# Vincentqyw/image-matching-webui

Measured on AMD Instinct MI355X. Metric: image-pairs/sec @640x480 SuperPoint+LightGlue, higher is better.
Workload: dtype f32 via 3xf16 split MFMA, f32 accumulate; P.V of LightGlue's cross blocks in two products (audited per block: layer error <= 7.1e-6, score error <= 4.7e-5, profiles/r05_lab_attention_mix.txt)

## Files before the change

image-matching-webui_amd/csrc/api.hip:

```cpp
#include <stdarg.h>
#include <stdio.h>
#include <stdlib.h>
#include <string.h>

#include "attention.h"
#include "conv.h"
#include "ffn.h"
#include "gemm.h"
#include "imcui_hip.h"

int imcui_set_err(imcui_hip_s* h, int code, const char* fmt, ...) {
    if (h) {
        va_list ap;
        va_start(ap, fmt);
        vsnprintf(h->err, sizeof h->err, fmt, ap);
        va_end(ap);
    }
    return code;
}

extern "C" int imcui_hip_version(void) { return 400; }

static const char* const OPT_NAMES[OPT_NCNT] = {"gemm_wreg", "wreg_pipe", "attn_variant", "attn_variant_self", "attn_variant_cross", "attn_mix_layers", "conv_tall", "conv_narrow", "simred", "ffn_tile", "wreg_tile", "attn_split", "loftr_fine_sparse"};
static int opt_index(const char* name) {
    if (!name) return -1;
    for (int i = 0; i < OPT_NCNT; ++i)
        if (strcmp(name, OPT_NAMES[i]) == 0) return i;
    return -1;
}
extern "C" int imcui_hip_set_option(imcui_hip_t* h, const char* name, int value) {
    const int i = opt_index(name);
    if (!h || i < 0) return imcui_set_err(h, IMCUI_ERR_ARG, "set_option: unknown option '%s'", name ? name : "(null)");
    h->opt[i] = value;
    return IMCUI_OK;
}
extern "C" int imcui_hip_get_option(imcui_hip_t* h, const char* name, int* value) {
    const int i = opt_index(name);
    if (!h || !value || i < 0) return imcui_set_err(h, IMCUI_ERR_ARG, "get_option: unknown option '%s'", name ? name : "(null)");
    *value = h->opt[i];
    return IMCUI_OK;
}

extern "C" int imcui_hip_create(int device, imcui_hip_t** out) {
    if (!out) return IMCUI_ERR_ARG;
    *out = nullptr;
    int n = 0;
    if (hipGetDeviceCount(&n) != hipSuccess || device < 0 || device >= n) return IMCUI_ERR_HIP;
    hipDeviceProp_t prop;
    if (hipGetDeviceProperties(&prop, device) != hipSuccess) return IMCUI_ERR_HIP;
    imcui_hip_s* h = (imcui_hip_s*)calloc(1, sizeof(imcui_hip_s));
    if (!h) return IMCUI_ERR_ARG;
    h->device = device;
    h->num_cu = prop.multiProcessorCount;
    h->err[0] = 0;
    h->precision = 1;
    {
        const char* e;
        h->opt[OPT_GEMM_WREG] = (e = getenv("IMCUI_GEMM_WREG")) ? atoi(e) : 2;
        h->opt[OPT_WREG_PIPE] = (e = getenv("IMCUI_WREG_PIPE")) ? atoi(e) : 1;
        h->opt[OPT_ATTN_VARIANT] = (e = getenv("IMCUI_ATTN_VARIANT")) ? atoi(e) : 8;
        h->opt[OPT_SIMRED] = (e = getenv("IMCUI_SIMRED")) ? atoi(e) : 1;
        h->opt[OPT_FFN_TILE] = (e = getenv("IMCUI_FFN_TILE")) ? atoi(e) : 0;
        h->opt[OPT_WREG_TILE] = (e = getenv("IMCUI_WREG_TILE")) ? atoi(e) : 0;
        h->opt[OPT_CONV_TALL] = (e = getenv("IMCUI_CONV_TALL")) ? atoi(e) : 1;
        h->opt[OPT_CONV_NARROW] = (e = getenv("IMCUI_CONV_NARROW")) ? atoi(e) : 0;
        h->opt[OPT_ATTN_SELF] = (e = getenv("IMCUI_ATTN_VARIANT_SELF")) ? atoi(e) : -1;
        h->opt[OPT_ATTN_CROSS] = (e = getenv("IMCUI_ATTN_VARIANT_CROSS")) ? atoi(e) : -2;
        h->opt[OPT_ATTN_SPLIT] = (e = getenv("IMCUI_ATTN_SPLIT")) ? atoi(e) : 1;
        h->opt[OPT_LOFTR_FINE_SPARSE] = (e = getenv("IMCUI_LOFTR_FINE_SPARSE")) ? atoi(e) : 1;
        h->opt[OPT_ATTN_MIX_LAYERS] = (e = getenv("IMCUI_ATTN_MIX_LAYERS")) ? (int)strtol(e, nullptr, 0) : 0x1ff;
    }
    *out = h;
    const char* rc = getenv("IMCUI_HIP_CHECK_RANGE");
    if (rc && atoi(rc) != 0) (void)imcui_hip_set_range_check(h, 1);
    return IMCUI_OK;
}

__global__ __launch_bounds__(256) void range_check_kernel(const float* __restrict__ x, long rows, int cols, long ld, const int* __restrict__ cnt,
                                                          int rows_per_seq, int* __restrict__ flag) {
    int bits = 0;
    const long n4 = rows * (long)(cols >> 2);
    for (long t = (long)blockIdx.x * 256 + threadIdx.x; t < n4; t += (long)gridDim.x * 256) {
        const long r = t / (cols >> 2);
        const int c = (int)(t - r * (cols >> 2)) * 4;
        if (cnt != nullptr && rows_per_seq > 0 && (int)(r % rows_per_seq) >= cnt[r / rows_per_seq]) continue;
        const float4 v = *reinterpret_cast<const float4*>(x + r * ld + c);
        const float a[4] = {v.x, v.y, v.z, v.w};
#pragma unroll
        for (int j = 0; j < 4; ++j) {
            if (!(fabsf(a[j]) <= 3.4028234e38f)) bits |= 2;
            else if (fabsf(a[j]) > 65504.0f) bits |= 1;
        }
    }
    if (bits) atomicOr(flag, bits);
}
void imcui_range_check(imcui_hip_s* h, const float* x, long rows, int cols, long ld, const int* cnt, int rows_per_seq, hipStream_t s) {
    if (!h || !h->range_flag || !x || rows <= 0 || cols < 4 || (cols & 3) || (ld & 3)) return;
    const long n4 = rows * (long)(cols >> 2);
// ... 540 lines not shown
```

image-matching-webui_amd/csrc/common.h:

```cpp
#pragma once
#include <hip/hip_runtime.h>
#include <stdint.h>

#include <atomic>

typedef float f32x16 __attribute__((ext_vector_type(16)));
typedef float f32x4 __attribute__((ext_vector_type(4)));

#define IMCUI_WAVE 64

__device__ __forceinline__ f32x16 mfma32(float a, float b, f32x16 c) {
    return __builtin_amdgcn_mfma_f32_32x32x2f32(a, b, c, 0, 0, 0);
}

typedef _Float16 f16x8 __attribute__((ext_vector_type(8)));
typedef _Float16 f16x2 __attribute__((ext_vector_type(2)));
typedef __fp16 fp16x2_t __attribute__((ext_vector_type(2)));

__device__ __forceinline__ f32x16 mfma16(uint4 a, uint4 b, f32x16 c) {
    return __builtin_amdgcn_mfma_f32_32x32x16_f16(__builtin_bit_cast(f16x8, a), __builtin_bit_cast(f16x8, b), c, 0, 0, 0);
}
__device__ __forceinline__ void split2(float x0, float x1, unsigned& hi, unsigned& lo) {
    const fp16x2_t h = __builtin_amdgcn_cvt_pkrtz(x0, x1);
    hi = __builtin_bit_cast(unsigned, h);
// ... 79 lines not shown
    int dev = 0;
    (void)hipGetDevice(&dev);
    const unsigned long long bit = 1ull << (dev & 63);
    if (done.load(std::memory_order_acquire) & bit) return true;
    if (hipFuncSetAttribute(kernel, hipFuncAttributeMaxDynamicSharedMemorySize, bytes) != hipSuccess) return false;
    done.fetch_or(bit, std::memory_order_release);
    return true;
}
static inline int cdiv(int a, int b) { return (a + b - 1) / b; }
static inline size_t align_up(size_t v, size_t a) { return (v + a - 1) / a * a; }
static inline unsigned blocks_256(long n) { return (unsigned)((n + 255) / 256); }
static inline unsigned grid_stride_blocks(long n) { return (n + 255) / 256 < 65536 ? blocks_256(n) : 65536u; }

#define IMCUI_OK 0
#define IMCUI_ERR_ARG -1
#define IMCUI_ERR_WS -2
#define IMCUI_ERR_HIP -3
#define IMCUI_ERR_UNSUPPORTED -4

enum {
    OPT_GEMM_WREG = 0,
    OPT_WREG_PIPE,
    OPT_ATTN_VARIANT,
    OPT_ATTN_SELF,
    OPT_ATTN_CROSS,
    OPT_ATTN_MIX_LAYERS,
    OPT_CONV_TALL,
    OPT_CONV_NARROW,
    OPT_SIMRED,
    OPT_FFN_TILE,
    OPT_WREG_TILE,
    OPT_ATTN_SPLIT,
    OPT_LOFTR_FINE_SPARSE,
    OPT_NCNT
};

#define IMCUI_GEMM_ROUTE_SLOTS 384
#define IMCUI_ATTN_ROUTE_SLOTS 16
#define IMCUI_CONV_ROUTE_SLOTS 16
#define IMCUI_FFN_ROUTE_SLOTS 17

enum { PROF_ATTN = 0, PROF_CONV = 1, PROF_GEMM = 2, PROF_NCLS = 3 };
#define PROF_MAX_EVENTS 4096
struct imcui_hip_s {
    int device;
    int num_cu;
    char err[512];
    int precision;
    int prof_on;
    int prof_used[PROF_NCLS];
    int prof_alloc[PROF_NCLS];
    hipEvent_t* prof_ev[PROF_NCLS];
    float* lg_dump;
    size_t lg_dump_floats;
    long long* ffn_dbg;
    int* range_flag;
    int opt[OPT_NCNT];
    int loftr_fine_mode;
    int loftr_fine_matches;
    int gemm_last_route;
    int gemm_route_count[IMCUI_GEMM_ROUTE_SLOTS];
    int gemm_route_features[IMCUI_GEMM_ROUTE_SLOTS];
    int attn_last_route;
    int attn_route_count[IMCUI_ATTN_ROUTE_SLOTS];
    int conv_last_route;
    int conv_route_count[IMCUI_CONV_ROUTE_SLOTS];
// ... 39 lines not shown
```

image-matching-webui_amd/csrc/conv.hip:

```cpp
#include <stdlib.h>

#include "conv.h"
#include "gemm.h"

#define TH 8
#define TW 16
#define PW (TW + 2)
#define PH (TH + 2)
#define NPIX (PH * PW)
#define PSTR 181
#define WSTR 65

__global__ __launch_bounds__(256) void conv3x3_kernel(const float* __restrict__ in, const float* __restrict__ wp,
                                                      const float* __restrict__ bias, float* __restrict__ out, int H,
                                                      int W, int Cin, int Cout, int tiles_x, int tiles_y, int relu,
                                                      int pool) {
    __shared__ float4 Ps[8 * PSTR];
    __shared__ float4 Ws[2][8 * WSTR];

    const int tid = threadIdx.x, lane = tid & 63, wid = tid >> 6;
    const int lo = lane & 31, hi = lane >> 5;
    const int ncout = Cout >> 6;
    const int t = xcd_remap(blockIdx.x, gridDim.x);
    const int ct = t % ncout;
// ... 81 lines not shown
            }
        }
    }
}

int conv3x3_launch(imcui_hip_s* h, const float* in, const float* wp, const float* bias, float* out, int B, int H, int W,
                   int Cin, int Cout, int relu, int pool, hipStream_t stream) {
    h->conv_last_route = CONV_ROUTE(CR_NONE);
    if (Cin % 32 != 0 || Cout % 64 != 0)
        return imcui_set_err(h, IMCUI_ERR_ARG, "conv3x3: Cin=%d must be a multiple of 32, Cout=%d of 64", Cin, Cout);
    if (pool && ((H | W) & 1)) return imcui_set_err(h, IMCUI_ERR_ARG, "conv3x3: pooled layer needs even H,W (%dx%d)", H, W);
    const int tiles_x = cdiv(W, TW), tiles_y = cdiv(H, TH);
    const long nwg = (long)tiles_x * tiles_y * (Cout / 64) * B;
    if (nwg <= 0) return IMCUI_OK;
    imcui_prof_begin(h, PROF_CONV, stream);
    hipLaunchKernelGGL(conv3x3_kernel, dim3((unsigned)nwg), dim3(256), 0, stream, in, wp, bias, out, H, W, Cin, Cout,
                       tiles_x, tiles_y, relu, pool);
    conv_route_note(h, CR_F32, pool ? CF_POOL : 0);
    imcui_prof_end(h, PROF_CONV, stream);
    IMCUI_CHECK_LAUNCH(h);
    return IMCUI_OK;
}

#define STH 8
#define STW 32
#define SPW (STW + 2)
#define SNPIX ((STH + 2) * SPW)
#define SPSTR 346

#define ITW (STW + 4)
#define ITH (STH + 4)
__device__ __forceinline__ float conv_act(float v, int code) { return code == 2 ? (v > 0.0f ? v : 0.01f * v) : (code == 1 ? fmaxf(v, 0.0f) : v); }

template <bool FUSE1A, int NC, bool SINGLE = false>
__global__ __launch_bounds__(256, NC == 4 ? 2 : 3) void conv3x3_split_kernel(const float* __restrict__ in,
                                                            const unsigned short* __restrict__ wh,
                                                            const unsigned short* __restrict__ wl,
                                                            const float* __restrict__ wscale,
                                                            const float* __restrict__ bias, float* __restrict__ out,
                                                            int H, int W, int Cin, int Cout, int tiles_x, int tiles_y,
                                                            int relu, int pool, const float* __restrict__ w1a,
                                                            const float* __restrict__ b1a, int cin_stride, int cout_live, ConvHead hd) {
    constexpr int WSN = NC * 32 + 1;
    static_assert(NC == 2 || (NC == 4 && !FUSE1A), "the fused first layer has 64 output channels");
    __shared__ uint4 smem[2 * 4 * SPSTR + 2 * 2 * 4 * WSN + (FUSE1A ? (ITH * ITW + 9 * 64 + 64 + 3) / 4 + 1 : 0)];
    uint4* Ph = smem;
    uint4* Pl = smem + 4 * SPSTR;
    uint4* Wb = smem + 2 * 4 * SPSTR;
    float* img = reinterpret_cast<float*>(smem + 2 * 4 * SPSTR + 2 * 2 * 4 * WSN);
    float* w1 = img + ITH * ITW;

    const int tid = threadIdx.x, lane = tid & 63, wid = tid >> 6;
    const int lo = lane & 31, hi = lane >> 5;
    const int ncout = Cout / (32 * NC);
    const int t = xcd_remap(blockIdx.x, gridDim.x);
    const int ct = t % ncout;
    int sp = t / ncout;
    const int tx = sp % tiles_x;
    sp /= tiles_x;
    const int ty = sp % tiles_y;
    const int b = sp / tiles_y;
    const int y0 = ty * STH, x0 = tx * STW, cout0 = ct * 32 * NC;
    const int nlive = min(NC, (cout_live - cout0 + 31) >> 5);
    const bool relu_in = !FUSE1A && (relu & 4) != 0;
    relu &= 3;

    f32x16 acc[2][NC];
#pragma unroll
    for (int m = 0; m < 2; ++m)
#pragma unroll
        for (int n = 0; n < NC; ++n)
#pragma unroll
            for (int r = 0; r < 16; ++r) acc[m][n][r] = 0.0f;

    const int nchunk = Cin >> 5;
    const uint4* wh4 = reinterpret_cast<const uint4*>(wh);
    const uint4* wl4 = reinterpret_cast<const uint4*>(wl);

    if (FUSE1A) {
        for (int i = tid; i < ITH * ITW; i += 256) {
            const int gy = y0 - 2 + i / ITW, gx = x0 - 2 + i % ITW;
            img[i] = (gy >= 0 && gy < H && gx >= 0 && gx < W) ? in[((size_t)b * H + gy) * W + gx] : 0.0f;
        }
        for (int i = tid; i < 9 * 64; i += 256) w1[i] = w1a[i];
        if (tid < 64) w1[9 * 64 + tid] = b1a[tid];
    }

    constexpr int NPG = (SNPIX * 4 + 255) / 256;
    float4 pa[NPG], pc[NPG];
    unsigned pvalid = 0;
    auto patch_fetch = [&](int ch) __attribute__((always_inline)) {
        pvalid = 0;
#pragma unroll
        for (int k = 0; k < NPG; ++k) {
            const int idx = tid + 256 * k;
            const int oc = idx & 3, pp = idx >> 2;
            const int py = pp / SPW, px = pp - py * SPW;
            const int gy = y0 - 1 + py, gx = x0 - 1 + px;
            if (idx < SNPIX * 4 && gy >= 0 && gy < H && gx >= 0 && gx < W) {
                const float* src = in + (((size_t)b * H + gy) * W + gx) * cin_stride + ch * 32 + oc * 8;
                pa[k] = *reinterpret_cast<const float4*>(src);
                pc[k] = *reinterpret_cast<const float4*>(src + 4);
                pvalid |= 1u << k;
            }
        }
    };
    auto patch_store = [&]() __attribute__((always_inline)) {
#pragma unroll
        for (int k = 0; k < NPG; ++k) {
            const int idx = tid + 256 * k;
            if (idx < SNPIX * 4) {
                uint4 hq = make_uint4(0u, 0u, 0u, 0u), lq = hq;
                if ((pvalid >> k) & 1u) {
                    if (relu_in) {
                        pa[k] = make_float4(fmaxf(pa[k].x, 0.f), fmaxf(pa[k].y, 0.f), fmaxf(pa[k].z, 0.f), fmaxf(pa[k].w, 0.f));
                        pc[k] = make_float4(fmaxf(pc[k].x, 0.f), fmaxf(pc[k].y, 0.f), fmaxf(pc[k].z, 0.f), fmaxf(pc[k].w, 0.f));
                    }
                    if constexpr (SINGLE)
                        hq = half8_rtn(pa[k], pc[k]);
                    else
                        split8(pa[k], pc[k], hq, lq);
                }
                Ph[(idx & 3) * SPSTR + (idx >> 2)] = hq;
                if constexpr (!SINGLE) Pl[(idx & 3) * SPSTR + (idx >> 2)] = lq;
            }
        }
    };
    constexpr bool PREFETCH = (NC == 2);
    if (!FUSE1A && PREFETCH) patch_fetch(0);

    for (int ch = 0; ch < nchunk; ++ch) {
        if (!FUSE1A && !PREFETCH) patch_fetch(ch);
        __syncthreads();
        if (!FUSE1A) {
            patch_store();
            if (PREFETCH && ch + 1 < nchunk) patch_fetch(ch + 1);
        }
        float4 kw0[9], kw1[9], kb0, kb1;
        if (FUSE1A) {
            const int c0 = ch * 32 + (tid & 3) * 8;
            kb0 = *reinterpret_cast<const float4*>(w1 + 9 * 64 + c0);
            kb1 = *reinterpret_cast<const float4*>(w1 + 9 * 64 + c0 + 4);
#pragma unroll
            for (int t9 = 0; t9 < 9; ++t9) {
                kw0[t9] = *reinterpret_cast<const float4*>(w1 + t9 * 64 + c0);
                kw1[t9] = *reinterpret_cast<const float4*>(w1 + t9 * 64 + c0 + 4);
            }
        }
        for (int idx = tid; FUSE1A && idx < SNPIX * 4; idx += 256) {
            const int oc = idx & 3, pp = idx >> 2;
            const int py = pp / SPW, px = pp - py * SPW;
            const int gy = y0 - 1 + py, gx = x0 - 1 + px;
            uint4 hq = make_uint4(0u, 0u, 0u, 0u), lq = hq;
            if (gy >= 0 && gy < H && gx >= 0 && gx < W) {
                float4 a, c;
                if (FUSE1A) {
                    a = kb0;
// ... 20 lines not shown
                    c = *reinterpret_cast<const float4*>(src + 4);
                }
                split8(a, c, hq, lq);
            }
            Ph[oc * SPSTR + pp] = hq;
            Pl[oc * SPSTR + pp] = lq;
        }
        uint4 rwh, rwl, rwh1, rwl1;
        auto wload = [&](int tap) __attribute__((always_inline)) {
            const size_t o = ((size_t)(ch * 9 + tap) * 4 + (tid >> 6)) * Cout + cout0 + (tid & 63);
            rwh = wh4[o];
            if constexpr (!SINGLE) rwl = wl4[o];
            if constexpr (NC == 4) {
                rwh1 = wh4[o + 64];
                if constexpr (!SINGLE) rwl1 = wl4[o + 64];
            }
        };
        wload(0);
        for (int tap = 0; tap < 9; ++tap) {
            uint4* wbh = Wb + (tap & 1) * (2 * 4 * WSN);
            uint4* wbl = wbh + 4 * WSN;
            wbh[(tid >> 6) * WSN + (tid & 63)] = rwh;
            if constexpr (!SINGLE) wbl[(tid >> 6) * WSN + (tid & 63)] = rwl;
            if constexpr (NC == 4) {
                wbh[(tid >> 6) * WSN + (tid & 63) + 64] = rwh1;
                if constexpr (!SINGLE) wbl[(tid >> 6) * WSN + (tid & 63) + 64] = rwl1;
            }
            __syncthreads();
            if (tap + 1 < 9) wload(tap + 1);
            const int dy = tap / 3, dx = tap - dy * 3;
#pragma unroll
            for (int st = 0; st < 2; ++st) {
                const int oc = 2 * st + hi;
                uint4 ah[2], al[2], bh[NC], bl[NC];
#pragma unroll
                for (int m = 0; m < 2; ++m) {
                    const int pp = (2 * wid + m + dy) * SPW + lo + dx;
                    ah[m] = Ph[oc * SPSTR + pp];
                    if constexpr (!SINGLE) al[m] = Pl[oc * SPSTR + pp];
                }
#pragma unroll
                for (int n = 0; n < NC; ++n) {
                    bh[n] = wbh[oc * WSN + n * 32 + lo];
                    if constexpr (!SINGLE) bl[n] = wbl[oc * WSN + n * 32 + lo];
                }
#pragma unroll
                for (int n = 0; n < NC; ++n) {
                    if (NC == 4 && n == NC - 1 && nlive < NC) break;
#pragma unroll
                    for (int m = 0; m < 2; ++m) {
                        if constexpr (!SINGLE) {
                            acc[m][n] = mfma16(bh[n], al[m], acc[m][n]);
                            acc[m][n] = mfma16(bl[n], ah[m], acc[m][n]);
                        }
                        acc[m][n] = mfma16(bh[n], ah[m], acc[m][n]);
                    }
                }
            }
        }
    }

    const float wsc = wscale[0];
    const float* resid = FUSE1A ? nullptr : w1a;
    const float* resid2 = FUSE1A ? nullptr : b1a;
    const bool late = resid != nullptr;
    __syncthreads();
    float* st = reinterpret_cast<float*>(smem);
    constexpr int SROW = 68;
#pragma unroll
    for (int half = 0; half < NC / 2; ++half) {
        const int coutH = cout0 + 64 * half;
        if (half > 0) __syncthreads();
        if (pool) {
            const int Ho = H >> 1, Wo = W >> 1;
#pragma unroll
            for (int n = 0; n < 2; ++n)
#pragma unroll
                for (int q = 0; q < 4; ++q) {
                    const int cl = n * 32 + 8 * q + 4 * hi;
                    const float4 b4 = *reinterpret_cast<const float4*>(bias + coutH + cl);
                    float v[4];
#pragma unroll
                    for (int j = 0; j < 4; ++j) {
                        float tv = fmaxf(acc[0][2 * half + n][4 * q + j], acc[1][2 * half + n][4 * q + j]);
                        tv = fmaxf(tv, __shfl_xor(tv, 1, 64));
                        v[j] = tv * wsc;
                    }
                    v[0] += b4.x;
                    v[1] += b4.y;
                    v[2] += b4.z;
                    v[3] += b4.w;
                    if (relu) {
#pragma unroll
                        for (int j = 0; j < 4; ++j) v[j] = conv_act(v[j], relu);
                    }
                    if ((lo & 1) == 0) *reinterpret_cast<float4*>(st + (wid * 16 + (lo >> 1)) * SROW + cl) = make_float4(v[0], v[1], v[2], v[3]);
                }
            __syncthreads();
#pragma unroll
            for (int it = 0; it < 4; ++it) {
                const int px = (tid >> 4) + 16 * it, c4 = tid & 15;
                const int oy = (y0 >> 1) + (px >> 4), pxo = (x0 >> 1) + (px & 15);
                if (oy < Ho && pxo < Wo)
                    *reinterpret_cast<float4*>(out + (((size_t)b * Ho + oy) * Wo + pxo) * Cout + coutH + 4 * c4) =
                        *reinterpret_cast<const float4*>(st + px * SROW + 4 * c4);
            }
        } else {
#pragma unroll
            for (int h2 = 0; h2 < 2; ++h2) {
                if ((wid >> 1) == h2) {
#pragma unroll
                    for (int n = 0; n < 2; ++n)
#pragma unroll
                        for (int q = 0; q < 4; ++q) {
                            const int cl = n * 32 + 8 * q + 4 * hi;
                            const float4 b4 = *reinterpret_cast<const float4*>(bias + coutH + cl);
#pragma unroll
                            for (int m = 0; m < 2; ++m) {
                                float4 v = make_float4(acc[m][2 * half + n][4 * q + 0] * wsc + b4.x, acc[m][2 * half + n][4 * q + 1] * wsc + b4.y,
                                                       acc[m][2 * half + n][4 * q + 2] * wsc + b4.z, acc[m][2 * half + n][4 * q + 3] * wsc + b4.w);
                                if (relu && !late) {
                                    v.x = conv_act(v.x, relu);
                                    v.y = conv_act(v.y, relu);
                                    v.z = conv_act(v.z, relu);
                                    v.w = conv_act(v.w, relu);
                                }
                                *reinterpret_cast<float4*>(st + (((wid & 1) * 2 + m) * 32 + lo) * SROW + cl) = v;
                            }
                        }
                }
                __syncthreads();
                if constexpr (NC == 4 && !FUSE1A) {
                    if (hd.w != nullptr) {
                        const int c4 = tid & 15;
                        float4 hw[4];
#pragma unroll
                        for (int c = 0; c < 4; ++c) hw[c] = *reinterpret_cast<const float4*>(hd.w + c * 128 + 64 * half + 4 * c4);
                        float* psum = st + 128 * SROW;
#pragma unroll
                        for (int it = 0; it < 8; ++it) {
                            const int px = (tid >> 4) + 16 * it;
                            const float4 v = *reinterpret_cast<const float4*>(st + px * SROW + 4 * c4);
                            float d[4];
#pragma unroll
                            for (int c = 0; c < 4; ++c) {
                                d[c] = (v.x * hw[c].x + v.y * hw[c].y) + (v.z * hw[c].z + v.w * hw[c].w);
#pragma unroll
                                for (int o = 8; o > 0; o >>= 1) d[c] += __shfl_xor(d[c], o, 64);
                            }
                            if (c4 == 0) {
                                float4* ps = reinterpret_cast<float4*>(psum + (h2 * 128 + px) * 4);
                                if (half == 0) {
                                    *ps = make_float4(d[0], d[1], d[2], d[3]);
                                } else {
                                    const float4 q = *ps;
                                    const int oy = y0 + 4 * h2 + (px >> 5), ox = x0 + (px & 31);
                                    if (oy < H && ox < W) {
                                        const float x = (q.x + d[0]) + hd.b[0], y = (q.y + d[1]) + hd.b[1], z = (q.z + d[2]) + hd.b[2], cf = (q.w + d[3]) + hd.b[3];
                                        const size_t p = ((size_t)b * H + oy) * W + ox;
                                        if (hd.raw) *reinterpret_cast<float4*>(hd.raw + p * 4) = make_float4(x, y, z, cf);
                                        const float dn = sqrtf(x * x + y * y + z * z);
                                        const float sc = expm1f(dn) / fmaxf(dn, 1e-8f);
                                        hd.pts[p * 3 + 0] = x * sc;
                                        hd.pts[p * 3 + 1] = y * sc;
                                        hd.pts[p * 3 + 2] = z * sc;
                                        hd.conf[p] = 1.0f + expf(cf);
                                    }
                                }
                            }
                        }
                    }
                }
#pragma unroll
                for (int it = 0; it < 8; ++it) {
                    const int px = (tid >> 4) + 16 * it, c4 = tid & 15;
                    const int oy = y0 + 4 * h2 + (px >> 5), ox = x0 + (px & 31);
                    if (oy < H && ox < W && out != nullptr) {
                        float4 v = *reinterpret_cast<const float4*>(st + px * SROW + 4 * c4);
                        const size_t o = (((size_t)b * H + oy) * W + ox) * Cout + coutH + 4 * c4;
                        if (late) {
                            float4 r4 = *reinterpret_cast<const float4*>(resid + o);
                            v = make_float4(v.x + r4.x, v.y + r4.y, v.z + r4.z, v.w + r4.w);
                            if (resid2) {
                                r4 = *reinterpret_cast<const float4*>(resid2 + o);
                                v = make_float4(v.x + r4.x, v.y + r4.y, v.z + r4.z, v.w + r4.w);
                            }
                            v = make_float4(conv_act(v.x, relu), conv_act(v.y, relu), conv_act(v.z, relu), conv_act(v.w, relu));
                        }
                        *reinterpret_cast<float4*>(out + o) = v;
                    }
                }
                if (h2 == 0) __syncthreads();
            }
        }
    }
}

#define TTH 16
#define TNPIX ((TTH + 2) * SPW)
#define TPSTR 618
#define TITH (TTH + 4)

template <bool FUSE1A, bool SINGLE = false>
__global__ __launch_bounds__(256, 2) void conv3x3_tall_kernel(const float* __restrict__ in, const unsigned short* __restrict__ wh,
                                                              const unsigned short* __restrict__ wl, const float* __restrict__ wscale,
                                                              const float* __restrict__ bias, float* __restrict__ out, int H, int W, int Cin,
                                                              int Cout, int tiles_x, int tiles_y, int relu, int pool,
                                                              const float* __restrict__ w1a, const float* __restrict__ b1a, int cin_stride) {
    constexpr int WSN = 65;
    __shared__ uint4 smem[2 * 2 * TPSTR + 2 * 2 * 2 * WSN + (FUSE1A ? (TITH * ITW + 9 * 64 + 64 + 3) / 4 + 1 : 0)];
    uint4* Ph = smem;
    uint4* Pl = smem + 2 * TPSTR;
    uint4* Wb = smem + 4 * TPSTR;
    float* img = reinterpret_cast<float*>(smem + 4 * TPSTR + 8 * WSN);
    float* w1 = img + TITH * ITW;

    const int tid = threadIdx.x, lane = tid & 63, wid = tid >> 6;
    const int lo = lane & 31, hi = lane >> 5;
    const int ncout = Cout >> 6;
    const int t = xcd_remap(blockIdx.x, gridDim.x);
    const int ct = t % ncout;
    int sp = t / ncout;
    const int tx = sp % tiles_x;
    sp /= tiles_x;
    const int ty = sp % tiles_y;
    const int b = sp / tiles_y;
    const int y0 = ty * TTH, x0 = tx * STW, cout0 = ct * 64;
    const bool relu_in = !FUSE1A && (relu & 4) != 0;
    relu &= 3;

    f32x16 acc[4][2];
#pragma unroll
    for (int m = 0; m < 4; ++m)
#pragma unroll
        for (int n = 0; n < 2; ++n)
#pragma unroll
            for (int r = 0; r < 16; ++r) acc[m][n][r] = 0.0f;

    const int nstage = Cin >> 4;
    const uint4* wh4 = reinterpret_cast<const uint4*>(wh);
    const uint4* wl4 = reinterpret_cast<const uint4*>(wl);

    if (FUSE1A) {
        for (int i = tid; i < TITH * ITW; i += 256) {
            const int gy = y0 - 2 + i / ITW, gx = x0 - 2 + i % ITW;
            img[i] = (gy >= 0 && gy < H && gx >= 0 && gx < W) ? in[((size_t)b * H + gy) * W + gx] : 0.0f;
        }
        for (int i = tid; i < 9 * 64; i += 256) w1[i] = w1a[i];
        if (tid < 64) w1[9 * 64 + tid] = b1a[tid];
    }

    constexpr int NPG = (TNPIX * 2 + 255) / 256;
    for (int cs = 0; cs < nstage; ++cs) {
        float4 pa[NPG], pc[NPG];
        unsigned pvalid = 0;
        if (!FUSE1A) {
#pragma unroll
            for (int k = 0; k < NPG; ++k) {
                const int idx = tid + 256 * k;
                const int oc = idx & 1, pp = idx >> 1;
                const int py = pp / SPW, px = pp - py * SPW;
                const int gy = y0 - 1 + py, gx = x0 - 1 + px;
                if (idx < TNPIX * 2 && gy >= 0 && gy < H && gx >= 0 && gx < W) {
                    const float* src = in + (((size_t)b * H + gy) * W + gx) * cin_stride + cs * 16 + oc * 8;
                    pa[k] = *reinterpret_cast<const float4*>(src);
                    pc[k] = *reinterpret_cast<const float4*>(src + 4);
                    pvalid |= 1u << k;
                }
            }
        }
        __syncthreads();
        if (!FUSE1A) {
#pragma unroll
            for (int k = 0; k < NPG; ++k) {
                const int idx = tid + 256 * k;
                if (idx < TNPIX * 2) {
                    uint4 hq = make_uint4(0u, 0u, 0u, 0u), lq = hq;
                    if ((pvalid >> k) & 1u) {
                        if (relu_in) {
                            pa[k] = make_float4(fmaxf(pa[k].x, 0.f), fmaxf(pa[k].y, 0.f), fmaxf(pa[k].z, 0.f), fmaxf(pa[k].w, 0.f));
                            pc[k] = make_float4(fmaxf(pc[k].x, 0.f), fmaxf(pc[k].y, 0.f), fmaxf(pc[k].z, 0.f), fmaxf(pc[k].w, 0.f));
                        }
                        if constexpr (SINGLE)
                            hq = half8_rtn(pa[k], pc[k]);
                        else
                            split8(pa[k], pc[k], hq, lq);
                    }
                    Ph[(idx & 1) * TPSTR + (idx >> 1)] = hq;
                    if constexpr (!SINGLE) Pl[(idx & 1) * TPSTR + (idx >> 1)] = lq;
                }
            }
        } else {
// ... 5 lines not shown
            for (int t9 = 0; t9 < 9; ++t9) {
                kw0[t9] = *reinterpret_cast<const float4*>(w1 + t9 * 64 + c0);
                kw1[t9] = *reinterpret_cast<const float4*>(w1 + t9 * 64 + c0 + 4);
            }
            for (int idx = tid; idx < TNPIX * 2; idx += 256) {
                const int oc = idx & 1, pp = idx >> 1;
                const int py = pp / SPW, px = pp - py * SPW;
                const int gy = y0 - 1 + py, gx = x0 - 1 + px;
                uint4 hq = make_uint4(0u, 0u, 0u, 0u), lq = hq;
                if (gy >= 0 && gy < H && gx >= 0 && gx < W) {
                    float4 a = kb0, c = kb1;
#pragma unroll
                    for (int t9 = 0; t9 < 9; ++t9) {
                        const float v = img[(py + t9 / 3) * ITW + px + t9 % 3];
                        const float4 k0 = kw0[t9];
                        const float4 k1 = kw1[t9];
                        a.x = fmaf(v, k0.x, a.x);
                        a.y = fmaf(v, k0.y, a.y);
                        a.z = fmaf(v, k0.z, a.z);
                        a.w = fmaf(v, k0.w, a.w);
                        c.x = fmaf(v, k1.x, c.x);
                        c.y = fmaf(v, k1.y, c.y);
                        c.z = fmaf(v, k1.z, c.z);
                        c.w = fmaf(v, k1.w, c.w);
                    }
                    a.x = fmaxf(a.x, 0.f); a.y = fmaxf(a.y, 0.f); a.z = fmaxf(a.z, 0.f); a.w = fmaxf(a.w, 0.f);
                    c.x = fmaxf(c.x, 0.f); c.y = fmaxf(c.y, 0.f); c.z = fmaxf(c.z, 0.f); c.w = fmaxf(c.w, 0.f);
                    split8(a, c, hq, lq);
                }
                Ph[oc * TPSTR + pp] = hq;
                Pl[oc * TPSTR + pp] = lq;
            }
        }
        uint4 rw;
        const int wplane = tid >> 7, woct = (tid >> 6) & 1, wc = tid & 63;
        auto wload = [&](int tap) __attribute__((always_inline)) {
            const size_t o = ((size_t)((cs >> 1) * 9 + tap) * 4 + (cs & 1) * 2 + woct) * Cout + cout0 + wc;
            if (wplane == 0)
                rw = wh4[o];
            else if constexpr (!SINGLE)
                rw = wl4[o];
        };
        wload(0);
        for (int tap = 0; tap < 9; ++tap) {
            uint4* wb = Wb + (tap & 1) * (4 * WSN);
            if (!SINGLE || wplane == 0) wb[wplane * (2 * WSN) + woct * WSN + wc] = rw;
            __syncthreads();
            if (tap + 1 < 9) wload(tap + 1);
            const int dy = tap / 3, dx = tap - dy * 3;
            const uint4* wbh = wb + hi * WSN;
            const uint4* wbl = wb + 2 * WSN + hi * WSN;
            uint4 ah[4], al[4], bh[2], bl[2];
#pragma unroll
            for (int m = 0; m < 4; ++m) {
                const int pp = (4 * wid + m + dy) * SPW + lo + dx;
                ah[m] = Ph[hi * TPSTR + pp];
                if constexpr (!SINGLE) al[m] = Pl[hi * TPSTR + pp];
            }
#pragma unroll
            for (int n = 0; n < 2; ++n) {
                bh[n] = wbh[n * 32 + lo];
                if constexpr (!SINGLE) bl[n] = wbl[n * 32 + lo];
            }
#pragma unroll
            for (int n = 0; n < 2; ++n)
#pragma unroll
                for (int m = 0; m < 4; ++m) {
                    if constexpr (!SINGLE) {
                        acc[m][n] = mfma16(bh[n], al[m], acc[m][n]);
                        acc[m][n] = mfma16(bl[n], ah[m], acc[m][n]);
                    }
                    acc[m][n] = mfma16(bh[n], ah[m], acc[m][n]);
                }
        }
    }

    const float wsc = wscale[0];
    const float* resid = FUSE1A ? nullptr : w1a;
    const float* resid2 = FUSE1A ? nullptr : b1a;
    const bool late = resid != nullptr;
    __syncthreads();
    float* st = reinterpret_cast<float*>(smem);
    constexpr int SROW = 68;
    if (pool) {
        const int Ho = H >> 1, Wo = W >> 1;
#pragma unroll
        for (int mp = 0; mp < 2; ++mp)
#pragma unroll
            for (int n = 0; n < 2; ++n)
#pragma unroll
                for (int q = 0; q < 4; ++q) {
                    const int cl = n * 32 + 8 * q + 4 * hi;
                    const float4 b4 = *reinterpret_cast<const float4*>(bias + cout0 + cl);
                    float v[4];
#pragma unroll
                    for (int j = 0; j < 4; ++j) {
                        float tv = fmaxf(acc[2 * mp][n][4 * q + j], acc[2 * mp + 1][n][4 * q + j]);
                        tv = fmaxf(tv, __shfl_xor(tv, 1, 64));
                        v[j] = tv * wsc;
                    }
                    v[0] += b4.x;
                    v[1] += b4.y;
                    v[2] += b4.z;
                    v[3] += b4.w;
                    if (relu) {
#pragma unroll
// ... 73 lines not shown
    if (pool && resid) return imcui_set_err(h, IMCUI_ERR_ARG, "conv3x3: residual input and fused pooling are exclusive");
    if (resid2 && !resid) return imcui_set_err(h, IMCUI_ERR_ARG, "conv3x3: a second residual map needs the first");
    if (head && (Cout != 128 || pool || resid || (relu & 3) != 1 || cout_live != Cout || !head->w || !head->b || !head->pts || !head->conf ||
                 conv_narrow_env(h)))
        return imcui_set_err(h, IMCUI_ERR_ARG, "conv3x3: the fused point-map head needs a 128-channel ReLU layer without pooling / residual");
    if (!head && !out) return imcui_set_err(h, IMCUI_ERR_ARG, "conv3x3: null output");
    if (Cin % 32 != 0 || Cout % 64 != 0)
        return imcui_set_err(h, IMCUI_ERR_ARG, "conv3x3: Cin=%d must be a multiple of 32, Cout=%d of 64", Cin, Cout);
    if (pool && ((H | W) & 1)) return imcui_set_err(h, IMCUI_ERR_ARG, "conv3x3: pooled layer needs even H,W (%dx%d)", H, W);
    const int feat = (pool ? CF_POOL : 0) | (resid ? CF_RESID : 0) | (resid2 ? CF_RESID2 : 0) | ((relu & 3) == 2 ? CF_LEAKY : 0) | ((relu & 4) ? CF_RELU_IN : 0) |
                     (cin_stride != Cin ? CF_CIN_STRIDE : 0) | (cout_live < Cout ? CF_COUT_LIVE : 0) |
                     (head ? CF_HEAD | (out ? 0 : CF_HEAD_NO_OUT) | (head->raw ? CF_HEAD_RAW : 0) : 0);
    const int tiles_x = cdiv(W, STW);
    bool narrow_only = conv_narrow_env(h);
    if (h->opt[OPT_CONV_NARROW] == 0 && !head && Cout % 128 == 0 && (long)tiles_x * cdiv(H, STH) * (Cout / 128) * B < 256) narrow_only = true;
    const bool wide = (Cout % 128 == 0) && !narrow_only;
    if (!wide && cout_live == Cout && conv_tall_mode(h) >= 2) {
        const int tiles_t = cdiv(H, TTH);
        const long nwg_t = (long)tiles_x * tiles_t * (Cout / 64) * B;
        if (nwg_t <= 0) return IMCUI_OK;
        if (h->range_flag) imcui_range_check(h, in, (long)B * H * W, Cin, cin_stride, nullptr, 0, stream);
        imcui_prof_begin(h, PROF_CONV, stream);
        if (single)
            hipLaunchKernelGGL((conv3x3_tall_kernel<false, true>), dim3((unsigned)nwg_t), dim3(256), 0, stream, in, wh, wl, wscale, bias, out, H, W, Cin, Cout,
                               tiles_x, tiles_t, relu, pool, resid, resid2, cin_stride);
        else
            hipLaunchKernelGGL((conv3x3_tall_kernel<false>), dim3((unsigned)nwg_t), dim3(256), 0, stream, in, wh, wl, wscale, bias, out, H, W, Cin, Cout,
                               tiles_x, tiles_t, relu, pool, resid, resid2, cin_stride);
        conv_route_note(h, single ? CR_TALL_SINGLE : CR_TALL, feat);
        imcui_prof_end(h, PROF_CONV, stream);
        IMCUI_CHECK_LAUNCH(h);
        return IMCUI_OK;
    }
    const int tiles_y = cdiv(H, STH);
    const long nwg = (long)tiles_x * tiles_y * (Cout / (wide ? 128 : 64)) * B;
    if (nwg <= 0) return IMCUI_OK;
    if (h->range_flag) imcui_range_check(h, in, (long)B * H * W, Cin, cin_stride, nullptr, 0, stream);
    imcui_prof_begin(h, PROF_CONV, stream);
    if (wide && single)
        hipLaunchKernelGGL((conv3x3_split_kernel<false, 4, true>), dim3((unsigned)nwg), dim3(256), 0, stream, in, wh, wl, wscale, bias, out, H, W, Cin, Cout,
                           tiles_x, tiles_y, relu, pool, resid, resid2, cin_stride, cout_live, head ? *head : ConvHead{});
    else if (single)
        hipLaunchKernelGGL((conv3x3_split_kernel<false, 2, true>), dim3((unsigned)nwg), dim3(256), 0, stream, in, wh, wl, wscale, bias, out, H, W, Cin, Cout,
                           tiles_x, tiles_y, relu, pool, resid, resid2, cin_stride, cout_live, head ? *head : ConvHead{});
    else if (wide)
        hipLaunchKernelGGL((conv3x3_split_kernel<false, 4>), dim3((unsigned)nwg), dim3(256), 0, stream, in, wh, wl, wscale, bias, out, H, W, Cin, Cout,
                           tiles_x, tiles_y, relu, pool, resid, resid2, cin_stride, cout_live, head ? *head : ConvHead{});
    else
        hipLaunchKernelGGL((conv3x3_split_kernel<false, 2>), dim3((unsigned)nwg), dim3(256), 0, stream, in, wh, wl, wscale, bias, out, H, W, Cin, Cout,
                           tiles_x, tiles_y, relu, pool, resid, resid2, cin_stride, cout_live, head ? *head : ConvHead{});
    conv_route_note(h, wide ? (single ? CR_SPLIT_N4_SINGLE : CR_SPLIT_N4) : (single ? CR_SPLIT_N2_SINGLE : CR_SPLIT_N2), feat);
    imcui_prof_end(h, PROF_CONV, stream);
    IMCUI_CHECK_LAUNCH(h);
    return IMCUI_OK;
}

int conv1ab_fused_split_launch(imcui_hip_s* h, const float* image, const float* w1a, const float* b1a,
                               const unsigned short* wh, const unsigned short* wl, const float* wscale, const float* bias,
                               float* out, int B, int H, int W, int pool, hipStream_t stream) {
    h->conv_last_route = CONV_ROUTE(CR_NONE);
    if (pool && ((H | W) & 1)) return imcui_set_err(h, IMCUI_ERR_ARG, "conv1ab: pooled layer needs even H,W (%dx%d)", H, W);
    const bool tall = conv_tall_mode(h) >= 1;
    const int tiles_x = cdiv(W, STW), tiles_y = cdiv(H, tall ? TTH : STH);
    const long nwg = (long)tiles_x * tiles_y * B;
    if (nwg <= 0) return IMCUI_OK;
    imcui_prof_begin(h, PROF_CONV, stream);
// ... 108 lines not shown
```

Before: 1028.

## Add alternative conv tile geometries: 16x16 fragments and three rows per wave

After: 1035, median of 6. About the same (+0.7%).

```diff
diff --git a/image-matching-webui_amd/csrc/api.hip b/image-matching-webui_amd/csrc/api.hip
--- a/image-matching-webui_amd/csrc/api.hip
+++ b/image-matching-webui_amd/csrc/api.hip
@@ -21,7 +21,7 @@
 
 extern "C" int imcui_hip_version(void) { return 400; }
 
-static const char* const OPT_NAMES[OPT_NCNT] = {"gemm_wreg", "wreg_pipe", "attn_variant", "attn_variant_self", "attn_variant_cross", "attn_mix_layers", "conv_tall", "conv_narrow", "simred", "ffn_tile", "wreg_tile", "attn_split", "loftr_fine_sparse"};
+static const char* const OPT_NAMES[OPT_NCNT] = {"gemm_wreg", "wreg_pipe", "attn_variant", "attn_variant_self", "attn_variant_cross", "attn_mix_layers", "conv_tall", "conv_narrow", "simred", "ffn_tile", "wreg_tile", "attn_split", "loftr_fine_sparse", "conv_geom"};
 static int opt_index(const char* name) {
     if (!name) return -1;
     for (int i = 0; i < OPT_NCNT; ++i)
@@ -64,6 +64,7 @@
         h->opt[OPT_WREG_TILE] = (e = getenv("IMCUI_WREG_TILE")) ? atoi(e) : 0;
         h->opt[OPT_CONV_TALL] = (e = getenv("IMCUI_CONV_TALL")) ? atoi(e) : 1;
         h->opt[OPT_CONV_NARROW] = (e = getenv("IMCUI_CONV_NARROW")) ? atoi(e) : 0;
+        h->opt[OPT_CONV_GEOM] = (e = getenv("IMCUI_CONV_GEOM")) ? atoi(e) : 1;
         h->opt[OPT_ATTN_SELF] = (e = getenv("IMCUI_ATTN_VARIANT_SELF")) ? atoi(e) : -1;
         h->opt[OPT_ATTN_CROSS] = (e = getenv("IMCUI_ATTN_VARIANT_CROSS")) ? atoi(e) : -2;
         h->opt[OPT_ATTN_SPLIT] = (e = getenv("IMCUI_ATTN_SPLIT")) ? atoi(e) : 1;
diff --git a/image-matching-webui_amd/csrc/common.h b/image-matching-webui_amd/csrc/common.h
--- a/image-matching-webui_amd/csrc/common.h
+++ b/image-matching-webui_amd/csrc/common.h
@@ -135,6 +135,7 @@
     OPT_WREG_TILE,
     OPT_ATTN_SPLIT,
     OPT_LOFTR_FINE_SPARSE,
+    OPT_CONV_GEOM,
     OPT_NCNT
 };
 
diff --git a/image-matching-webui_amd/csrc/conv.hip b/image-matching-webui_amd/csrc/conv.hip
--- a/image-matching-webui_amd/csrc/conv.hip
+++ b/image-matching-webui_amd/csrc/conv.hip
@@ -137,8 +137,8 @@
 #define ITH (STH + 4)
 __device__ __forceinline__ float conv_act(float v, int code) { return code == 2 ? (v > 0.0f ? v : 0.01f * v) : (code == 1 ? fmaxf(v, 0.0f) : v); }
 
-template <bool FUSE1A, int NC, bool SINGLE = false>
-__global__ __launch_bounds__(256, NC == 4 ? 2 : 3) void conv3x3_split_kernel(const float* __restrict__ in,
+template <bool FUSE1A, int NC, bool SINGLE = false, bool G16 = false, int MR = 2>
+__global__ __launch_bounds__(256, (NC == 4 || MR == 3) ? 2 : 3) void conv3x3_split_kernel(const float* __restrict__ in,
                                                             const unsigned short* __restrict__ wh,
                                                             const unsigned short* __restrict__ wl,
                                                             const float* __restrict__ wscale,
@@ -148,11 +148,18 @@
                                                             const float* __restrict__ b1a, int cin_stride, int cout_live, ConvHead hd) {
     constexpr int WSN = NC * 32 + 1;
     static_assert(NC == 2 || (NC == 4 && !FUSE1A), "the fused first layer has 64 output channels");
-    __shared__ uint4 smem[2 * 4 * SPSTR + 2 * 2 * 4 * WSN + (FUSE1A ? (ITH * ITW + 9 * 64 + 64 + 3) / 4 + 1 : 0)];
+    static_assert(!(G16 && FUSE1A), "the fused first layer keeps the 32-column fragments");
+    static_assert(MR == 2 || (MR == 3 && NC == 2 && !FUSE1A && !G16 && !SINGLE), "three rows per wave: the plain 64-channel instance");
+    constexpr int TH_ = G16 ? 16 : 4 * MR, TW_ = G16 ? 16 : STW;
+    constexpr int PSTR_ = MR == 3 ? 490 : SPSTR;
+    constexpr int PW_ = TW_ + 2, NPIX_ = (TH_ + 2) * PW_;
+    constexpr int FR = G16 ? 2 : 1;
+    static_assert(NPIX_ <= PSTR_ - 6, "the patch must fit the LDS carve");
+    __shared__ uint4 smem[2 * 4 * PSTR_ + 2 * 2 * 4 * WSN + (FUSE1A ? (ITH * ITW + 9 * 64 + 64 + 3) / 4 + 1 : 0)];
     uint4* Ph = smem;
-    uint4* Pl = smem + 4 * SPSTR;
-    uint4* Wb = smem + 2 * 4 * SPSTR;
-    float* img = reinterpret_cast<float*>(smem + 2 * 4 * SPSTR + 2 * 2 * 4 * WSN);
+    uint4* Pl = smem + 4 * PSTR_;
+    uint4* Wb = smem + 2 * 4 * PSTR_;
+    float* img = reinterpret_cast<float*>(smem + 2 * 4 * PSTR_ + 2 * 2 * 4 * WSN);
     float* w1 = img + ITH * ITW;
 
     const int tid = threadIdx.x, lane = tid & 63, wid = tid >> 6;
@@ -165,14 +172,15 @@
     sp /= tiles_x;
     const int ty = sp % tiles_y;
     const int b = sp / tiles_y;
-    const int y0 = ty * STH, x0 = tx * STW, cout0 = ct * 32 * NC;
+    const int y0 = ty * TH_, x0 = tx * TW_, cout0 = ct * 32 * NC;
+    const int frow = G16 ? lo >> 4 : 0, fcol = G16 ? (lo - 2 * (lo >> 4)) & 15 : lo;
     const int nlive = min(NC, (cout_live - cout0 + 31) >> 5);
     const bool relu_in = !FUSE1A && (relu & 4) != 0;
     relu &= 3;
 
-    f32x16 acc[2][NC];
-#pragma unroll
-    for (int m = 0; m < 2; ++m)
+    f32x16 acc[MR][NC];
+#pragma unroll
+    for (int m = 0; m < MR; ++m)
 #pragma unroll
         for (int n = 0; n < NC; ++n)
 #pragma unroll
@@ -191,7 +199,7 @@
         if (tid < 64) w1[9 * 64 + tid] = b1a[tid];
     }
 
-    constexpr int NPG = (SNPIX * 4 + 255) / 256;
+    constexpr int NPG = (NPIX_ * 4 + 255) / 256;
     float4 pa[NPG], pc[NPG];
     unsigned pvalid = 0;
     auto patch_fetch = [&](int ch) __attribute__((always_inline)) {
@@ -200,9 +208,9 @@
         for (int k = 0; k < NPG; ++k) {
             const int idx = tid + 256 * k;
             const int oc = idx & 3, pp = idx >> 2;
-            const int py = pp / SPW, px = pp - py * SPW;
+            const int py = pp / PW_, px = pp - py * PW_;
             const int gy = y0 - 1 + py, gx = x0 - 1 + px;
-            if (idx < SNPIX * 4 && gy >= 0 && gy < H && gx >= 0 && gx < W) {
+            if (idx < NPIX_ * 4 && gy >= 0 && gy < H && gx >= 0 && gx < W) {
                 const float* src = in + (((size_t)b * H + gy) * W + gx) * cin_stride + ch * 32 + oc * 8;
                 pa[k] = *reinterpret_cast<const float4*>(src);
                 pc[k] = *reinterpret_cast<const float4*>(src + 4);
@@ -214,7 +222,7 @@
 #pragma unroll
         for (int k = 0; k < NPG; ++k) {
             const int idx = tid + 256 * k;
-            if (idx < SNPIX * 4) {
+            if (idx < NPIX_ * 4) {
                 uint4 hq = make_uint4(0u, 0u, 0u, 0u), lq = hq;
                 if ((pvalid >> k) & 1u) {
                     if (relu_in) {
@@ -226,8 +234,8 @@
                     else
                         split8(pa[k], pc[k], hq, lq);
                 }
-                Ph[(idx & 3) * SPSTR + (idx >> 2)] = hq;
-                if constexpr (!SINGLE) Pl[(idx & 3) * SPSTR + (idx >> 2)] = lq;
+                Ph[(idx & 3) * PSTR_ + (idx >> 2)] = hq;
+                if constexpr (!SINGLE) Pl[(idx & 3) * PSTR_ + (idx >> 2)] = lq;
             }
         }
     };
@@ -314,12 +322,12 @@
 #pragma unroll
             for (int st = 0; st < 2; ++st) {
                 const int oc = 2 * st + hi;
-                uint4 ah[2], al[2], bh[NC], bl[NC];
-#pragma unroll
-                for (int m = 0; m < 2; ++m) {
-                    const int pp = (2 * wid + m + dy) * SPW + lo + dx;
-                    ah[m] = Ph[oc * SPSTR + pp];
-                    if constexpr (!SINGLE) al[m] = Pl[oc * SPSTR + pp];
+                uint4 ah[MR], al[MR], bh[NC], bl[NC];
+#pragma unroll
+                for (int m = 0; m < MR; ++m) {
+                    const int pp = ((MR * wid + m) * FR + frow + dy) * PW_ + fcol + dx;
+                    ah[m] = Ph[oc * PSTR_ + pp];
+                    if constexpr (!SINGLE) al[m] = Pl[oc * PSTR_ + pp];
                 }
 #pragma unroll
                 for (int n = 0; n < NC; ++n) {
@@ -330,7 +338,7 @@
                 for (int n = 0; n < NC; ++n) {
                     if (NC == 4 && n == NC - 1 && nlive < NC) break;
 #pragma unroll
-                    for (int m = 0; m < 2; ++m) {
+                    for (int m = 0; m < MR; ++m) {
                         if constexpr (!SINGLE) {
                             acc[m][n] = mfma16(bh[n], al[m], acc[m][n]);
                             acc[m][n] = mfma16(bl[n], ah[m], acc[m][n]);
@@ -349,12 +357,62 @@
     __syncthreads();
     float* st = reinterpret_cast<float*>(smem);
     constexpr int SROW = 68;
+    int erow = 0, ecol = lo, elane = lane;
+    if constexpr (G16) {
+        elane = (int)__lane_id();
+        erow = (elane >> 4) & 1;
+        ecol = (elane - 2 * erow) & 15;
+    }
 #pragma unroll
     for (int half = 0; half < NC / 2; ++half) {
         const int coutH = cout0 + 64 * half;
         if (half > 0) __syncthreads();
-        if (pool) {
+        if (pool && MR == 3) {
+            if constexpr (MR == 3) {
+                const int Ho = H >> 1, Wo = W >> 1;
+#pragma unroll
+                for (int m = 0; m < MR; ++m)
+#pragma unroll
+                    for (int n = 0; n < 2; ++n)
+#pragma unroll
+                        for (int q = 0; q < 4; ++q) {
+                            const int cl = n * 32 + 8 * q + 4 * hi;
+                            float v[4];
+#pragma unroll
+                            for (int j = 0; j < 4; ++j) {
+                                const float tv = acc[m][n][4 * q + j];
+                                v[j] = fmaxf(tv, __shfl_xor(tv, 1, 64));
+                            }
+                            if ((lo & 1) == 0) *reinterpret_cast<float4*>(st + ((MR * wid + m) * 16 + (lo >> 1)) * SROW + cl) = make_float4(v[0], v[1], v[2], v[3]);
+                        }
+                __syncthreads();
+#pragma unroll
+                for (int it = 0; it < 6; ++it) {
+                    const int px = (tid >> 4) + 16 * it, c4 = tid & 15;
+                    const int oy = (y0 >> 1) + (px >> 4), pxo = (x0 >> 1) + (px & 15);
+                    if (oy < Ho && pxo < Wo) {
+                        const float4 r0 = *reinterpret_cast<const float4*>(st + (2 * (px >> 4) * 16 + (px & 15)) * SROW + 4 * c4);
+                        const float4 r1 = *reinterpret_cast<const float4*>(st + ((2 * (px >> 4) + 1) * 16 + (px & 15)) * SROW + 4 * c4);
+                        const float4 b4 = *reinterpret_cast<const float4*>(bias + coutH + 4 * c4);
+                        float v[4] = {fmaxf(r0.x, r1.x), fmaxf(r0.y, r1.y), fmaxf(r0.z, r1.z), fmaxf(r0.w, r1.w)};
+#pragma unroll
+                        for (int j = 0; j < 4; ++j) v[j] = v[j] * wsc;
+                        v[0] += b4.x;
+                        v[1] += b4.y;
+                        v[2] += b4.z;
+                        v[3] += b4.w;
+                        if (relu) {
+#pragma unroll
+                            for (int j = 0; j < 4; ++j) v[j] = conv_act(v[j], relu);
+                        }
+                        *reinterpret_cast<float4*>(out + (((size_t)b * Ho + oy) * Wo + pxo) * Cout + coutH + 4 * c4) = make_float4(v[0], v[1], v[2], v[3]);
+                    }
+                }
+            }
+        } else if (pool) {
             const int Ho = H >> 1, Wo = W >> 1;
+#pragma unroll
+            for (int mp = 0; mp < (G16 ? 2 : 1); ++mp)
 #pragma unroll
             for (int n = 0; n < 2; ++n)
 #pragma unroll
@@ -364,7 +422,13 @@
                     float v[4];
 #pragma unroll
                     for (int j = 0; j < 4; ++j) {
-                        float tv = fmaxf(acc[0][2 * half + n][4 * q + j], acc[1][2 * half + n][4 * q + j]);
+                        float tv;
+                        if constexpr (G16) {
+                            tv = acc[mp][2 * half + n][4 * q + j];
+                            tv = fmaxf(tv, __shfl(tv, (elane & 32) + (erow ? (elane - 2) & 15 : 16 + ((elane + 2) & 15)), 64));
+                        } else {
+                            tv = fmaxf(acc[0][2 * half + n][4 * q + j], acc[1][2 * half + n][4 * q + j]);
+                        }
                         tv = fmaxf(tv, __shfl_xor(tv, 1, 64));
                         v[j] = tv * wsc;
                     }
@@ -376,21 +440,47 @@
 #pragma unroll
                         for (int j = 0; j < 4; ++j) v[j] = conv_act(v[j], relu);
                     }
-                    if ((lo & 1) == 0) *reinterpret_cast<float4*>(st + (wid * 16 + (lo >> 1)) * SROW + cl) = make_float4(v[0], v[1], v[2], v[3]);
+                    if constexpr (G16) {
+                        if ((lo & 17) == 0) *reinterpret_cast<float4*>(st + ((2 * wid + mp) * 8 + (lo >> 1)) * SROW + cl) = make_float4(v[0], v[1], v[2], v[3]);
+                    } else {
+                        if ((lo & 1) == 0) *reinterpret_cast<float4*>(st + (wid * 16 + (lo >> 1)) * SROW + cl) = make_float4(v[0], v[1], v[2], v[3]);
+                    }
                 }
             __syncthreads();
 #pragma unroll
             for (int it = 0; it < 4; ++it) {
                 const int px = (tid >> 4) + 16 * it, c4 = tid & 15;
-                const int oy = (y0 >> 1) + (px >> 4), pxo = (x0 >> 1) + (px & 15);
+                const int oy = (y0 >> 1) + (G16 ? px >> 3 : px >> 4), pxo = (x0 >> 1) + (G16 ? px & 7 : px & 15);
                 if (oy < Ho && pxo < Wo)
                     *reinterpret_cast<float4*>(out + (((size_t)b * Ho + oy) * Wo + pxo) * Cout + coutH + 4 * c4) =
                         *reinterpret_cast<const float4*>(st + px * SROW + 4 * c4);
             }
         } else {
 #pragma unroll
-            for (int h2 = 0; h2 < 2; ++h2) {
-                if ((wid >> 1) == h2) {
+            for (int h2 = 0; h2 < (G16 ? 2 : MR); ++h2) {
+                if constexpr (MR == 3) {
+#pragma unroll
+                    for (int m = 0; m < MR; ++m) {
+                        const int r = MR * wid + m;
+                        if ((r >> 2) != h2) continue;
+#pragma unroll
+                        for (int n = 0; n < 2; ++n)
+#pragma unroll
+                            for (int q = 0; q < 4; ++q) {
+                                const int cl = n * 32 + 8 * q + 4 * hi;
+                                const float4 b4 = *reinterpret_cast<const float4*>(bias + coutH + cl);
+                                float4 v = make_float4(acc[m][n][4 * q + 0] * wsc + b4.x, acc[m][n][4 * q + 1] * wsc + b4.y, acc[m][n][4 * q + 2] * wsc + b4.z,
+                                                       acc[m][n][4 * q + 3] * wsc + b4.w);
+                                if (relu && !late) {
+                                    v.x = conv_act(v.x, relu);
+                                    v.y = conv_act(v.y, relu);
+                                    v.z = conv_act(v.z, relu);
+                                    v.w = conv_act(v.w, relu);
+                                }
+                                *reinterpret_cast<float4*>(st + ((r & 3) * 32 + lo) * SROW + cl) = v;
+                            }
+                    }
+                } else if ((wid >> 1) == h2) {
 #pragma unroll
                     for (int n = 0; n < 2; ++n)
 #pragma unroll
@@ -407,12 +497,12 @@
                                     v.z = conv_act(v.z, relu);
                                     v.w = conv_act(v.w, relu);
                                 }
-                                *reinterpret_cast<float4*>(st + (((wid & 1) * 2 + m) * 32 + lo) * SROW + cl) = v;
+                                *reinterpret_cast<float4*>(st + (((wid & 1) * 2 + m) * 32 + erow * 16 + ecol) * SROW + cl) = v;
                             }
                         }
                 }
                 __syncthreads();
-                if constexpr (NC == 4 && !FUSE1A) {
+                if constexpr (NC == 4 && !FUSE1A && !G16) {
                     if (hd.w != nullptr) {
                         const int c4 = tid & 15;
                         float4 hw[4];
@@ -456,7 +546,7 @@
 #pragma unroll
                 for (int it = 0; it < 8; ++it) {
                     const int px = (tid >> 4) + 16 * it, c4 = tid & 15;
-                    const int oy = y0 + 4 * h2 + (px >> 5), ox = x0 + (px & 31);
+                    const int oy = y0 + (G16 ? 8 * h2 + (px >> 4) : 4 * h2 + (px >> 5)), ox = x0 + (px & (TW_ - 1));
                     if (oy < H && ox < W && out != nullptr) {
                         float4 v = *reinterpret_cast<const float4*>(st + px * SROW + 4 * c4);
                         const size_t o = (((size_t)b * H + oy) * W + ox) * Cout + coutH + 4 * c4;
@@ -472,7 +562,7 @@
                         *reinterpret_cast<float4*>(out + o) = v;
                     }
                 }
-                if (h2 == 0) __syncthreads();
+                if (h2 + 1 < (G16 ? 2 : MR)) __syncthreads();
             }
         }
     }
@@ -790,6 +880,42 @@
         IMCUI_CHECK_LAUNCH(h);
         return IMCUI_OK;
     }
+    const int geom = h->opt[OPT_CONV_GEOM], wrem = W % STW;
+    const bool g16 = !head && !single &&
+                     (geom == 2 || ((geom == 1 || geom == 4) && wrem >= 1 && wrem <= 16 && (long)cdiv(H, 16) * cdiv(W, 16) < (long)cdiv(H, STH) * tiles_x));
+    const bool rows3 = !g16 && !wide && !single &&
+                       (geom == 3 || ((geom == 1 || geom == 5) && pool && cdiv(H, 12) * 12 <= cdiv(H, STH) * STH &&
+                                      (long)tiles_x * cdiv(H, 12) * (Cout / 64) * B >= 2L * h->num_cu));
+    if (rows3) {
+        const int ty12 = cdiv(H, 12);
+        const long nwg12 = (long)tiles_x * ty12 * (Cout / 64) * B;
+        if (nwg12 <= 0) return IMCUI_OK;
+        if (h->range_flag) imcui_range_check(h, in, (long)B * H * W, Cin, cin_stride, nullptr, 0, stream);
+        imcui_prof_begin(h, PROF_CONV, stream);
+        hipLaunchKernelGGL((conv3x3_split_kernel<false, 2, false, false, 3>), dim3((unsigned)nwg12), dim3(256), 0, stream, in, wh, wl, wscale, bias, out, H, W, Cin,
+                           Cout, tiles_x, ty12, relu, pool, resid, resid2, cin_stride, cout_live, ConvHead{});
+        conv_route_note(h, CR_SPLIT_N2, feat);
+        imcui_prof_end(h, PROF_CONV, stream);
+        IMCUI_CHECK_LAUNCH(h);
+        return IMCUI_OK;
+    }
+    if (g16) {
+        const int tx16 = cdiv(W, 16), ty16 = cdiv(H, 16);
+        const long nwg16 = (long)tx16 * ty16 * (Cout / (wide ? 128 : 64)) * B;
+        if (nwg16 <= 0) return IMCUI_OK;
+        if (h->range_flag) imcui_range_check(h, in, (long)B * H * W, Cin, cin_stride, nullptr, 0, stream);
+        imcui_prof_begin(h, PROF_CONV, stream);
+        if (wide)
+            hipLaunchKernelGGL((conv3x3_split_kernel<false, 4, false, true>), dim3((unsigned)nwg16), dim3(256), 0, stream, in, wh, wl, wscale, bias, out, H, W, Cin,
+                               Cout, tx16, ty16, relu, pool, resid, resid2, cin_stride, cout_live, ConvHead{});
+        else
+            hipLaunchKernelGGL((conv3x3_split_kernel<false, 2, false, true>), dim3((unsigned)nwg16), dim3(256), 0, stream, in, wh, wl, wscale, bias, out, H, W, Cin,
+                               Cout, tx16, ty16, relu, pool, resid, resid2, cin_stride, cout_live, ConvHead{});
+        conv_route_note(h, wide ? CR_SPLIT_N4 : CR_SPLIT_N2, feat);
+        imcui_prof_end(h, PROF_CONV, stream);
+        IMCUI_CHECK_LAUNCH(h);
+        return IMCUI_OK;
+    }
     const int tiles_y = cdiv(H, STH);
     const long nwg = (long)tiles_x * tiles_y * (Cout / (wide ? 128 : 64)) * B;
     if (nwg <= 0) return IMCUI_OK;
```

## Restructure tall conv tap loop by column to reuse activation rows across dy

Applied to the files above, without the earlier changes.

Result: no change. 989.3 before, 998.8 after, median of 6 (+1.0%).

```diff
diff --git a/image-matching-webui_amd/csrc/conv.hip b/image-matching-webui_amd/csrc/conv.hip
--- a/image-matching-webui_amd/csrc/conv.hip
+++ b/image-matching-webui_amd/csrc/conv.hip
@@ -490,11 +490,11 @@
                                                               int Cout, int tiles_x, int tiles_y, int relu, int pool,
                                                               const float* __restrict__ w1a, const float* __restrict__ b1a, int cin_stride) {
     constexpr int WSN = 65;
-    __shared__ uint4 smem[2 * 2 * TPSTR + 2 * 2 * 2 * WSN + (FUSE1A ? (TITH * ITW + 9 * 64 + 64 + 3) / 4 + 1 : 0)];
+    __shared__ uint4 smem[2 * 2 * TPSTR + 2 * 3 * 2 * 2 * WSN + (FUSE1A ? (TITH * ITW + 9 * 64 + 64 + 3) / 4 + 1 : 0)];
     uint4* Ph = smem;
     uint4* Pl = smem + 2 * TPSTR;
     uint4* Wb = smem + 4 * TPSTR;
-    float* img = reinterpret_cast<float*>(smem + 4 * TPSTR + 8 * WSN);
+    float* img = reinterpret_cast<float*>(smem + 4 * TPSTR + 24 * WSN);
     float* w1 = img + TITH * ITW;
 
     const int tid = threadIdx.x, lane = tid & 63, wid = tid >> 6;
@@ -537,9 +537,11 @@
         float4 pa[NPG], pc[NPG];
         unsigned pvalid = 0;
         if (!FUSE1A) {
+            int ftid = tid;
+            asm volatile("" : "+v"(ftid));
 #pragma unroll
             for (int k = 0; k < NPG; ++k) {
-                const int idx = tid + 256 * k;
+                const int idx = ftid + 256 * k;
                 const int oc = idx & 1, pp = idx >> 1;
                 const int py = pp / SPW, px = pp - py * SPW;
                 const int gy = y0 - 1 + py, gx = x0 - 1 + px;
@@ -611,46 +613,61 @@
                 Pl[oc * TPSTR + pp] = lq;
             }
         }
-        uint4 rw;
+        uint4 rw0, rw1, rw2;
         const int wplane = tid >> 7, woct = (tid >> 6) & 1, wc = tid & 63;
-        auto wload = [&](int tap) __attribute__((always_inline)) {
-            const size_t o = ((size_t)((cs >> 1) * 9 + tap) * 4 + (cs & 1) * 2 + woct) * Cout + cout0 + wc;
-            if (wplane == 0)
-                rw = wh4[o];
-            else if constexpr (!SINGLE)
-                rw = wl4[o];
+        auto wload = [&](int dx) __attribute__((always_inline)) {
+            const size_t o = ((size_t)((cs >> 1) * 9 + dx) * 4 + (cs & 1) * 2 + woct) * Cout + cout0 + wc;
+            const size_t dyo = (size_t)3 * 4 * Cout;
+            if (wplane == 0) {
+                rw0 = wh4[o];
+                rw1 = wh4[o + dyo];
+                rw2 = wh4[o + 2 * dyo];
+            } else if constexpr (!SINGLE) {
+                rw0 = wl4[o];
+                rw1 = wl4[o + dyo];
+                rw2 = wl4[o + 2 * dyo];
+            }
         };
         wload(0);
-        for (int tap = 0; tap < 9; ++tap) {
-            uint4* wb = Wb + (tap & 1) * (4 * WSN);
-            if (!SINGLE || wplane == 0) wb[wplane * (2 * WSN) + woct * WSN + wc] = rw;
+#pragma unroll 1
+        for (int dx = 0; dx < 3; ++dx) {
+            uint4* wb = Wb + (dx & 1) * (3 * 4 * WSN);
+            if (!SINGLE || wplane == 0) {
+                uint4* wd = wb + wplane * (2 * WSN) + woct * WSN + wc;
+                wd[0] = rw0;
+                wd[4 * WSN] = rw1;
+                wd[8 * WSN] = rw2;
+            }
             __syncthreads();
-            if (tap + 1 < 9) wload(tap + 1);
-            const int dy = tap / 3, dx = tap - dy * 3;
-            const uint4* wbh = wb + hi * WSN;
-            const uint4* wbl = wb + 2 * WSN + hi * WSN;
-            uint4 ah[4], al[4], bh[2], bl[2];
-#pragma unroll
-            for (int m = 0; m < 4; ++m) {
-                const int pp = (4 * wid + m + dy) * SPW + lo + dx;
-                ah[m] = Ph[hi * TPSTR + pp];
-                if constexpr (!SINGLE) al[m] = Pl[hi * TPSTR + pp];
-            }
-#pragma unroll
-            for (int n = 0; n < 2; ++n) {
-                bh[n] = wbh[n * 32 + lo];
-                if constexpr (!SINGLE) bl[n] = wbl[n * 32 + lo];
-            }
-#pragma unroll
-            for (int n = 0; n < 2; ++n)
-#pragma unroll
-                for (int m = 0; m < 4; ++m) {
-                    if constexpr (!SINGLE) {
-                        acc[m][n] = mfma16(bh[n], al[m], acc[m][n]);
-                        acc[m][n] = mfma16(bl[n], ah[m], acc[m][n]);
-                    }
-                    acc[m][n] = mfma16(bh[n], ah[m], acc[m][n]);
-                }
+            if (dx + 1 < 3) wload(dx + 1);
+            uint4 ah[6], al[6];
+#pragma unroll
+            for (int r = 0; r < 6; ++r) {
+                const int pp = (4 * wid + r) * SPW + lo + dx;
+                ah[r] = Ph[hi * TPSTR + pp];
+                if constexpr (!SINGLE) al[r] = Pl[hi * TPSTR + pp];
+            }
+#pragma unroll
+            for (int dy = 0; dy < 3; ++dy) {
+                const uint4* wbh = wb + dy * (4 * WSN) + hi * WSN;
+                const uint4* wbl = wbh + 2 * WSN;
+                uint4 bh[2], bl[2];
+#pragma unroll
+                for (int n = 0; n < 2; ++n) {
+                    bh[n] = wbh[n * 32 + lo];
+                    if constexpr (!SINGLE) bl[n] = wbl[n * 32 + lo];
+                }
+#pragma unroll
+                for (int n = 0; n < 2; ++n)
+#pragma unroll
+                    for (int m = 0; m < 4; ++m) {
+                        if constexpr (!SINGLE) {
+                            acc[m][n] = mfma16(bh[n], al[m + dy], acc[m][n]);
+                            acc[m][n] = mfma16(bl[n], ah[m + dy], acc[m][n]);
+                        }
+                        acc[m][n] = mfma16(bh[n], ah[m + dy], acc[m][n]);
+                    }
+            }
         }
     }
 
```
